# jkrasting/momlevel

Hardware: AMD Instinct MI355X
Metric: Mcells/s for fused Wright-EOS+steric at 1440×1080×75; % HBM roofline (higher is better)
Workload: dtype f64

## Files before the change

momlevel_amd/csrc/build.py:

```python

import os
import shutil
import subprocess
import sys

HERE = os.path.dirname(os.path.abspath(__file__))
PKG = os.path.dirname(HERE)
ROOT = os.path.dirname(PKG)
_TIMED_UNITS = ["momlevel_hip.hip", "momlevel_promote.hip"]
FEATURES = {
    "strat": ["eos_device.hpp", "mlx_internal.hpp", "mlx_pack.hpp"],
    "trend": ["eos_device.hpp", "mlx_internal.hpp", "include/momlevel_trend.h"],
    "clim": ["eos_device.hpp", "mlx_internal.hpp", "mlx_pack.hpp", "include/momlevel_clim.h"],
    "gauge": ["eos_device.hpp", "mlx_internal.hpp", "include/momlevel_gauge.h"],
    "spice": ["mlx_internal.hpp", "include/momlevel_spice.h"],
    "vort": ["mlx_internal.hpp", "include/momlevel_vort.h"],
    "area": ["mlx_internal.hpp", "mlx_pack.hpp", "include/momlevel_area.h"],
    "layer": ["mlx_internal.hpp", "mlx_pack.hpp", "include/momlevel_layer.h"],
    "filter": ["eos_device.hpp", "mlx_internal.hpp", "mlx_pack.hpp", "include/momlevel_filter.h"],
    "quantile": ["eos_device.hpp", "mlx_internal.hpp", "mlx_pack.hpp",
                 "include/momlevel_quantile.h"],
}


def _path(name):
    return os.path.join(ROOT, name) if name.startswith("include/") else os.path.join(HERE, name)


def _feature_files(feature):
    return [_path(f"momlevel_{feature}.hip")] + [_path(name) for name in FEATURES[feature]]


SOURCES = [_path(name) for name in _TIMED_UNITS + [f"momlevel_{f}.hip" for f in FEATURES]
           + ["host_copy.cpp"]]
LIB = os.path.join(PKG, "libmomlevel_hip.so")

FLAGS = [
    "--offload-arch=gfx950",
    "-O3",
    "-ffp-contract=off",
    "-fPIC",
    "-shared",
    "-std=c++17",
    "-Wall",
    "-Wno-unused-variable",
    "-Wno-sometimes-uninitialized",
]


TIMED_SOURCES = [
    os.path.join(HERE, "momlevel_hip.hip"),
    os.path.join(HERE, "eos_device.hpp"),
    os.path.join(HERE, "mlx_internal.hpp"),
    os.path.join(HERE, "momlevel_promote.hip"),
    os.path.join(HERE, "eos_promote.hpp"),
    os.path.join(ROOT, "include", "momlevel_hip.h"),
    os.path.join(ROOT, "include", "momlevel_path.h"),
]
DEPENDS = sorted({*SOURCES, *TIMED_SOURCES, *(p for f in FEATURES for p in _feature_files(f)),
                  os.path.abspath(__file__)})


def source_sha(paths=None, flags=True):
    import hashlib

    h = hashlib.sha256()
    for path in (TIMED_SOURCES if paths is None else paths):
        with open(path, "rb") as f:
            h.update(f.read())
    if flags:
        h.update(" ".join(FLAGS).encode())
    return h.hexdigest()[:16]


def feature_source_sha(feature):
    return source_sha(_feature_files(feature))


def strat_source_sha():
    return feature_source_sha("strat")


def trend_source_sha():
    return feature_source_sha("trend")


def clim_source_sha():
    return feature_source_sha("clim")


def gauge_source_sha():
    return feature_source_sha("gauge")


def spice_source_sha():
    return feature_source_sha("spice")


def vort_source_sha():
    return feature_source_sha("vort")


def area_source_sha():
    return feature_source_sha("area")


def layer_source_sha():
    return feature_source_sha("layer")


def filter_source_sha():
    return feature_source_sha("filter")


def quantile_source_sha():
    return feature_source_sha("quantile")


def hipcc():
    exe = shutil.which("hipcc") or "/opt/rocm/bin/hipcc"
    if not os.path.exists(exe):
        raise RuntimeError("hipcc not found (looked on PATH and in /opt/rocm/bin)")
    return exe


def is_stale():
    if not os.path.exists(LIB):
        return True
    lib_mtime = os.path.getmtime(LIB)
    return any(os.path.getmtime(p) > lib_mtime for p in DEPENDS)


def build(force=False, verbose=False, extra_flags=()):
    if not force and not is_stale():
        return LIB
    cmd = [hipcc()] + FLAGS + list(extra_flags) + SOURCES + ["-o", LIB + ".tmp"]
    if verbose:
        print(" ".join(cmd), flush=True)
    res = subprocess.run(cmd, capture_output=True, text=True)
    if res.returncode != 0:
        raise RuntimeError(f"hipcc failed ({res.returncode}):\n{res.stdout}\n{res.stderr}")
    if verbose and res.stderr:
        print(res.stderr)
    os.replace(LIB + ".tmp", LIB)
    return LIB


if __name__ == "__main__":
    path = build(force="--force" in sys.argv, verbose=True)
    print(path)
```

momlevel_amd/csrc/momlevel_hip.hip:

```cpp

#include <hip/hip_runtime.h>
#include <stdint.h>
#include <stdio.h>
#include <string.h>

#include <initializer_list>
#include <type_traits>

#include "../../include/momlevel_hip.h"
#include "eos_device.hpp"
#include "mlx_internal.hpp"

#pragma clang fp contract(off)

namespace mlx {

constexpr int kBlock = 256;
constexpr int kNTC = 8;

template <typename TIn, int VEC>
struct Pack {
  TIn v[VEC];
};

typedef float f4_t __attribute__((ext_vector_type(4)));

template <bool STREAM>
__device__ __forceinline__ f4_t load16(const void* p) {
  if constexpr (STREAM) return __builtin_nontemporal_load(reinterpret_cast<const f4_t*>(p));
  else return *reinterpret_cast<const f4_t*>(p);
}

template <typename TIn, int VEC, bool STREAM = false>
__device__ __forceinline__ Pack<TIn, VEC> load_pack(const TIn* __restrict__ p) {
  Pack<TIn, VEC> r;
  if constexpr (VEC == 1) {
    if constexpr (STREAM) r.v[0] = __builtin_nontemporal_load(p);
    else r.v[0] = p[0];
  } else if constexpr (sizeof(TIn) * VEC == 8) {
    double raw;
    if constexpr (STREAM) raw = __builtin_nontemporal_load(reinterpret_cast<const double*>(p));
    else raw = *reinterpret_cast<const double*>(p);
    __builtin_memcpy(&r, &raw, 8);
  } else if constexpr (sizeof(TIn) * VEC == 16) {
    f4_t raw = load16<STREAM>(p);
    __builtin_memcpy(&r, &raw, 16);
  } else {
    static_assert(sizeof(TIn) * VEC == 32, "pack must be 16 or 32 bytes");
    f4_t raw0 = load16<STREAM>(p);
    f4_t raw1 = load16<STREAM>(reinterpret_cast<const char*>(p) + 16);
    __builtin_memcpy(&r.v[0], &raw0, 16);
    __builtin_memcpy(&r.v[VEC / 2], &raw1, 16);
  }
  return r;
}

template <int MODE, bool IS_T, typename TIn, int VEC, bool STREAM = false>
__device__ __forceinline__ Pack<TIn, VEC> load_field(const TIn* __restrict__ base, int64_t off) {
  constexpr bool F32_HERE = (MODE == kMixT32 && IS_T) || (MODE == kMixS32 && !IS_T);
  if constexpr (F32_HERE) {
    static_assert((VEC == 1 || VEC == 2) && sizeof(TIn) == 8, "the other field is float64");
    Pack<TIn, VEC> r;
    const float* q = reinterpret_cast<const float*>(base) + off;
    if constexpr (VEC == 2) {
      const Pack<float, 2> f = load_pack<float, 2, STREAM>(q);
      r.v[0] = f.v[0];
      r.v[1] = f.v[1];
    } else if constexpr (STREAM) {
      r.v[0] = __builtin_nontemporal_load(q);
    } else {
      r.v[0] = q[0];
    }
    return r;
  } else {
    return load_pack<TIn, VEC, STREAM>(base + off);
  }
}

__device__ __forceinline__ int64_t xcd_remap(int64_t b, int64_t n) {
  const int64_t q = n / 8, r = n % 8, xcd = b % 8, k = b / 8;
  return (xcd < r ? xcd * (q + 1) : r * (q + 1) + (xcd - r) * q) + k;
}

template <int VEC, bool STREAM = false>
__device__ __forceinline__ void store_pack(double* __restrict__ p, const Pack<double, VEC>& r) {
  if constexpr (VEC == 1) {
    if constexpr (STREAM) __builtin_nontemporal_store(r.v[0], p);
    else p[0] = r.v[0];
  } else {
#pragma unroll
    for (int h = 0; h < VEC / 2; ++h) {
      f4_t raw;
      __builtin_memcpy(&raw, &r.v[2 * h], 16);
      if constexpr (STREAM) __builtin_nontemporal_store(raw, reinterpret_cast<f4_t*>(p) + h);
      else reinterpret_cast<f4_t*>(p)[h] = raw;
    }
  }
}

template <int VEC, bool STREAM = false>
__device__ __forceinline__ void store_pack(float* __restrict__ p, const Pack<float, VEC>& r) {
  if constexpr (VEC == 1) {
    if constexpr (STREAM) __builtin_nontemporal_store(r.v[0], p);
    else p[0] = r.v[0];
  } else if constexpr (VEC == 2) {
    double raw;
    __builtin_memcpy(&raw, &r, 8);
    if constexpr (STREAM) __builtin_nontemporal_store(raw, reinterpret_cast<double*>(p));
    else *reinterpret_cast<double*>(p) = raw;
  } else {
    static_assert(VEC == 4, "float packs are 4, 8 or 16 bytes");
    f4_t raw;
    __builtin_memcpy(&raw, &r, 16);
    if constexpr (STREAM) __builtin_nontemporal_store(raw, reinterpret_cast<f4_t*>(p));
    else *reinterpret_cast<f4_t*>(p) = raw;
  }
}

__device__ __forceinline__ void lds_dma16(const void* gsrc, void* lds_slice) {
#if defined(__HIP_DEVICE_COMPILE__)
  __builtin_amdgcn_global_load_lds(gsrc, (__attribute__((address_space(3))) void*)lds_slice, 16, 0,
                                   2 );
#endif
}

__device__ __forceinline__ double wave_sum(double v) {
#pragma unroll
  for (int off = 32; off > 0; off >>= 1) v += __shfl_down(v, off, 64);
  return v;
}

constexpr int kVarSteric = 0, kVarHalo = 1, kVarThermo = 2, kVarAll = 3;

template <typename TIn, int VEC, int U, int VAR, int MODE, bool GENERIC, bool SKIP, bool FMA,
          bool P3D = false>
__global__ __launch_bounds__(kBlock) void k_steric_global(
    const TIn* __restrict__ T, const TIn* __restrict__ S, const TIn* __restrict__ T0,
    const TIn* __restrict__ S0, const double* __restrict__ vol0, const double* __restrict__ p,
    int p_mode, int eos, int nt, int t_chunk, int64_t plane, int64_t t_stride_T,
    int64_t t_stride_S, double* __restrict__ partials, int64_t nblk_total) {
  constexpr int NOUT = (VAR == kVarAll) ? 4 : 1;
  constexpr int NTC = (VAR == kVarAll) ? kNTC / 2 : kNTC;
  constexpr bool STREAM_T = (VAR != kVarHalo), STREAM_S = (VAR != kVarThermo);
  constexpr bool HELD_T = (VAR == kVarHalo || VAR == kVarAll);
  constexpr bool HELD_S = (VAR == kVarThermo || VAR == kVarAll);
  typedef typename PolyType<MODE>::type R;
  typedef typename PolyVec<MODE, GENERIC ? 1 : VEC>::type RV;
  constexpr int W = Lanes<RV>::n, G = VEC / W;
  constexpr bool GUARD = !GENERIC && VAR != kVarAll;
  constexpr bool PRED = !(VAR == kVarSteric && sizeof(TIn) == 8);
  typedef typename std::conditional<
      FMA, typename FusedFor<MODE>::type,
      typename std::conditional<GUARD, typename ExactFastFor<MODE>::type, ExactOps>::type>::type Ops;
  __shared__ double red[NOUT][NTC][kBlock];

  const int tid = threadIdx.x;
  const int z = blockIdx.y;
  const int nz = gridDim.y;
  const int tb = blockIdx.z * t_chunk;
  const int te = (tb + t_chunk < nt) ? (tb + t_chunk) : nt;
  const int64_t bx = xcd_remap(blockIdx.x, gridDim.x);
  const int64_t blk = (int64_t)blockIdx.y * gridDim.x + bx;
  const int64_t tile0 = bx * (kBlock * VEC * U);
  const int64_t zoff = (int64_t)z * plane;

  int64_t off[U];
  double vol[U][VEC];
  double pc[U][VEC];
  bool alive[U];
#pragma unroll
  for (int u = 0; u < U; ++u) {
    int64_t i = tile0 + ((int64_t)u * kBlock + tid) * VEC;
    const bool valid = (i + VEC <= plane);
    i = valid ? i : 0;
    off[u] = zoff + i;
    Pack<double, VEC> v = load_pack<double, VEC>(vol0 + off[u]);
    bool any_wet = false;
#pragma unroll
    for (int k = 0; k < VEC; ++k) {
      vol[u][k] = valid ? v.v[k] : canonical_nan();
      if constexpr (Ops::contracts && MLX_TUNE_FMA_ACC)
        vol[u][k] = (vol[u][k] == 0.0) ? canonical_nan() : vol[u][k];
      any_wet = any_wet || !is_nan(vol[u][k]);
    }
    alive[u] = !SKIP || any_wet;
    if ((GENERIC && p_mode == MLX_P_FULL3D) || P3D) {
      Pack<double, VEC> q = load_pack<double, VEC>(p + off[u]);
#pragma unroll
      for (int k = 0; k < VEC; ++k) pc[u][k] = q.v[k];
    }
  }
  static_assert(!(P3D && GENERIC), "P3D is the fast kernels' form of MLX_P_FULL3D");
  static_assert(!Ops::fused || W == 1, "pressure folding is per cell");
  double pz = 0.0;
  if ((!GENERIC && !P3D) || p_mode == MLX_P_ZPROF) pz = p[z];
  if (GENERIC && p_mode == MLX_P_SCALAR) pz = p[0];
  auto p_at = [&](int u, int k) -> double { return P3D ? pc[u][k] : pz; };
  auto pfold_at = [&](int u, int g) -> RV {
    RV f = RV{};
    if constexpr (Ops::fused) f = (R)p_at(u, g * W);
    return f;
  };
  lanemask_t pbad[U];
#pragma unroll
  for (int u = 0; u < U; ++u) {
    pbad[u] = P3D ? 0 : Ops::p_unsafe(pz);
    if constexpr (P3D) {
#pragma unroll
      for (int k = 0; k < VEC; ++k) pbad[u] |= Ops::p_unsafe_lanes(pc[u][k]);
    }
  }

  TPart<RV> t0p[(HELD_T && !GENERIC) ? U : 1][G];
  SPart<RV> s0p[(HELD_S && !GENERIC) ? U : 1][G];
  TIn t0v[(HELD_T && GENERIC) ? U : 1][VEC], s0v[(HELD_S && GENERIC) ? U : 1][VEC];
  if constexpr (HELD_T) {
#pragma unroll
    for (int u = 0; u < U; ++u) {
      Pack<TIn, VEC> h = {};
      if (alive[u]) h = load_field<MODE, true, TIn, VEC, true>(T0, off[u]);
#pragma unroll
      for (int k = 0; k < VEC; ++k) {
        if constexpr (GENERIC) t0v[u][k] = h.v[k];
      }
      if constexpr (!GENERIC) {
#pragma unroll
        for (int g = 0; g < G; ++g) t0p[u][g] = t_part_m<MODE, Ops, RV>(Lanes<RV>::make(&h.v[g * W]));
      }
    }
  }
  if constexpr (HELD_S) {
#pragma unroll
    for (int u = 0; u < U; ++u) {
      Pack<TIn, VEC> h = {};
      if (alive[u]) h = load_field<MODE, false, TIn, VEC, true>(S0, off[u]);
#pragma unroll
      for (int k = 0; k < VEC; ++k) {
        if constexpr (GENERIC) s0v[u][k] = h.v[k];
      }
      if constexpr (!GENERIC) {
#pragma unroll
        for (int g = 0; g < G; ++g)
          s0p[u][g] = s_part_m<MODE, Ops, RV>(Lanes<RV>::make(&h.v[g * W]), pfold_at(u, g));
      }
    }
  }

  constexpr bool PREFETCH = !(VAR == kVarAll && sizeof(TIn) == 8 && !GENERIC);
  constexpr bool GLDS = !PREFETCH && !IsMixed<MODE>::value;
  constexpr bool DIRECT = !PREFETCH && !GLDS;
  static_assert(!GLDS || sizeof(TIn) * VEC == 16, "one 16-byte LDS-DMA per pack");
  __shared__ f4_t stage[GLDS ? 2 * U : 1][kBlock];
  Pack<TIn, VEC> curT[U], curS[U], nxtT[PREFETCH ? U : 1], nxtS[PREFETCH ? U : 1];
  if constexpr (GLDS) {
#pragma unroll
    for (int u = 0; u < U; ++u) {
      if (alive[u]) {
        lds_dma16(T + (int64_t)tb * t_stride_T + off[u], &stage[u][tid & ~63]);
        lds_dma16(S + (int64_t)tb * t_stride_S + off[u], &stage[U + u][tid & ~63]);
      }
    }
  }
#pragma unroll
  for (int u = 0; u < (PREFETCH ? U : 0); ++u) {
    nxtT[u] = {};
    nxtS[u] = {};
    if (alive[u]) {
      if (STREAM_T) nxtT[u] = load_field<MODE, true, TIn, VEC, true>(T, (int64_t)tb * t_stride_T + off[u]);
      if (STREAM_S) nxtS[u] = load_field<MODE, false, TIn, VEC, true>(S, (int64_t)tb * t_stride_S + off[u]);
    }
  }

  for (int t = tb; t < te; ++t) {
    if constexpr (GLDS) {
      asm volatile("s_waitcnt vmcnt(0)" ::: "memory");
#pragma unroll
      for (int u = 0; u < U; ++u) {
        __builtin_memcpy(&curT[u], &stage[u][tid], 16);
        __builtin_memcpy(&curS[u], &stage[U + u][tid], 16);
      }
      asm volatile("s_waitcnt lgkmcnt(0)" ::: "memory");
      if (t + 1 < te) {
#pragma unroll
        for (int u = 0; u < U; ++u) {
          if (alive[u]) {
            lds_dma16(T + (int64_t)(t + 1) * t_stride_T + off[u], &stage[u][tid & ~63]);
            lds_dma16(S + (int64_t)(t + 1) * t_stride_S + off[u], &stage[U + u][tid & ~63]);
          }
        }
      }
    }
#pragma unroll
    for (int u = 0; u < (PREFETCH ? U : 0); ++u) {
      if (STREAM_T) curT[u] = nxtT[u];
      if (STREAM_S) curS[u] = nxtS[u];
    }
    if constexpr (DIRECT) {
#pragma unroll
      for (int u = 0; u < U; ++u) {
        curT[u] = {};
        curS[u] = {};
        if (alive[u]) {
          curT[u] = load_field<MODE, true, TIn, VEC, true>(T, (int64_t)t * t_stride_T + off[u]);
          curS[u] = load_field<MODE, false, TIn, VEC, true>(S, (int64_t)t * t_stride_S + off[u]);
        }
      }
    }
    if (PREFETCH && t + 1 < te) {
#pragma unroll
      for (int u = 0; u < U; ++u) {
        if (alive[u]) {
          if (STREAM_T)
            nxtT[u] = load_field<MODE, true, TIn, VEC, true>(T, (int64_t)(t + 1) * t_stride_T + off[u]);
          if (STREAM_S)
            nxtS[u] = load_field<MODE, false, TIn, VEC, true>(S, (int64_t)(t + 1) * t_stride_S + off[u]);
        }
      }
    }
    double c[NOUT];
#pragma unroll
    for (int o = 0; o < NOUT; ++o) c[o] = 0.0;
#pragma unroll
    for (int u = 0; u < U; ++u) {
      if (SKIP && !alive[u]) continue;
      constexpr int NR = NOUT > 1 ? 3 : 1;
      double rho[NR][VEC];
      if constexpr (GENERIC) {
#pragma unroll
        for (int k = 0; k < VEC; ++k) {
          double pp = pz;
          if (p_mode == MLX_P_FULL3D) pp = pc[u][k];
          if (p_mode == MLX_P_FULL4D) pp = p[((int64_t)t * nz) * plane + off[u] + k];
          const TIn tv = STREAM_T ? curT[u].v[k] : t0v[u][k];
          const TIn sv = STREAM_S ? curS[u].v[k] : s0v[u][k];
          rho[0][k] = eos_eval<MODE, TIn, Ops>(eos, kDensity, tv, sv, pp);
          if constexpr (VAR == kVarAll) {
            rho[1][k] = eos_eval<MODE, TIn, Ops>(eos, kDensity, tv, s0v[u][k], pp);
            rho[2][k] = eos_eval<MODE, TIn, Ops>(eos, kDensity, t0v[u][k], sv, pp);
          }
        }
      } else if constexpr (VAR == kVarAll) {
#pragma unroll
        for (int g = 0; g < G; ++g) {
          const TPart<RV> a = t_part_m<MODE, Ops, RV>(Lanes<RV>::make(&curT[u].v[g * W]));
          const SPart<RV> b = s_part_m<MODE, Ops, RV>(Lanes<RV>::make(&curS[u].v[g * W]), pfold_at(u, g));
          double r3[3][W];
          static_assert(!(P3D && VAR == kVarAll), "the all-variants kernel has no register to spare");
          wright_combine_lanes<Ops, RV>(a, b, pz, r3[0]);
          wright_combine_lanes<Ops, RV>(a, s0p[u][g], pz, r3[1]);
          wright_combine_lanes<Ops, RV>(t0p[u][g], b, pz, r3[2]);
#pragma unroll
          for (int w = 0; w < W; ++w) {
            const int k = g * W + w;
#pragma unroll
            for (int o = 0; o < 3; ++o) accumulate<Ops, PRED>(c[o], r3[o][w], vol[u][k]);
            accumulate<ExactOps, PRED>(c[3], (double)curT[u].v[k], vol[u][k]);
          }
        }
        continue;
      } else {
        double num[VEC], den[VEC];
#pragma unroll
        for (int g = 0; g < G; ++g) {
          TPart<RV> a;
          SPart<RV> b;
          if constexpr (STREAM_T) a = t_part_m<MODE, Ops, RV>(Lanes<RV>::make(&curT[u].v[g * W]));
          if constexpr (STREAM_S)
            b = s_part_m<MODE, Ops, RV>(Lanes<RV>::make(&curS[u].v[g * W]), pfold_at(u, g));
          double pg[W];
#pragma unroll
          for (int w = 0; w < W; ++w) pg[w] = p_at(u, g * W + w);
          if constexpr (VAR == kVarSteric)
            wright_numden_lanes<Ops, RV>(a, b, pg, &num[g * W], &den[g * W]);
          if constexpr (VAR == kVarHalo)
            wright_numden_lanes<Ops, RV>(t0p[u][g], b, pg, &num[g * W], &den[g * W]);
          if constexpr (VAR == kVarThermo)
            wright_numden_lanes<Ops, RV>(a, s0p[u][g], pg, &num[g * W], &den[g * W]);
        }
        quotients<Ops, VEC>(num, den, rho[0], pbad[u]);
      }
#pragma unroll
      for (int k = 0; k < VEC; ++k) {
#pragma unroll
        for (int o = 0; o < NR; ++o) accumulate<Ops, PRED>(c[o], rho[o][k], vol[u][k]);
        if constexpr (VAR == kVarAll)
          accumulate<ExactOps, PRED>(c[3], (double)curT[u].v[k], vol[u][k]);
      }
    }
    const int row = (t - tb) % NTC;
#pragma unroll
    for (int o = 0; o < NOUT; ++o) red[o][row][tid] = c[o];
    if (row == NTC - 1 || t == te - 1) {
      __syncthreads();
      const int wave = tid >> 6, lane = tid & 63;
      for (int q = wave; q < NOUT * (row + 1); q += kBlock / 64) {
        const int o = q / (row + 1), r = q % (row + 1);
        double v = ((red[o][r][lane] + red[o][r][lane + 64]) + red[o][r][lane + 128]) +
                   red[o][r][lane + 192];
        v = wave_sum(v);
        if (lane == 0) partials[((int64_t)o * nt + (t - row + r)) * nblk_total + blk] = v;
      }
      __syncthreads();
    }
  }
}

__global__ __launch_bounds__(kBlock) void k_reduce_rows(const double* __restrict__ partials,
                                                        int64_t n, double* __restrict__ out) {
  __shared__ double red[kBlock];
  const double* row = partials + (int64_t)blockIdx.x * n;
  double c = 0.0;
  int64_t i = threadIdx.x;
  for (; i + 7 * (int64_t)kBlock < n; i += 8 * (int64_t)kBlock) {
    double v[8];
#pragma unroll
    for (int k = 0; k < 8; ++k) v[k] = row[i + (int64_t)k * kBlock];
#pragma unroll
    for (int k = 0; k < 8; ++k) c += v[k];
  }
  for (; i < n; i += kBlock) c += row[i];
  red[threadIdx.x] = c;
  __syncthreads();
#pragma unroll
  for (int s = kBlock / 2; s > 0; s >>= 1) {
    if (threadIdx.x < s) red[threadIdx.x] += red[threadIdx.x + s];
    __syncthreads();
  }
  if (threadIdx.x == 0) out[blockIdx.x] = red[0];
}

__global__ __launch_bounds__(kBlock) void k_masso_partial(const double* __restrict__ rho,
                                                          const double* __restrict__ vol,
                                                          int64_t n3, int64_t vol_t_stride,
                                                          double* __restrict__ partials) {
  __shared__ double red[kBlock / 64];
  const int64_t t = blockIdx.y;
  const double* r = rho + t * n3;
  const double* v = vol + t * vol_t_stride;
  double c = 0.0;
  for (int64_t i = (int64_t)blockIdx.x * kBlock + threadIdx.x; i < n3;
       i += (int64_t)gridDim.x * kBlock) {
    const double term = r[i] * v[i];
    c += is_nan(term) ? 0.0 : term;
  }
  c = wave_sum(c);
  if ((threadIdx.x & 63) == 0) red[threadIdx.x >> 6] = c;
  __syncthreads();
  if (threadIdx.x == 0)
    partials[t * gridDim.x + blockIdx.x] = ((red[0] + red[1]) + red[2]) + red[3];
}

template <bool VEC2>
__global__ __launch_bounds__(kBlock) void k_nansum_partial(const double* __restrict__ x, int64_t n,
                                                           double* __restrict__ partials) {
  __shared__ double red[kBlock / 64];
  double c = 0.0;
  if constexpr (VEC2) {
    const int64_t n2 = n / 2;
    double c1 = 0.0;
    for (int64_t i = (int64_t)blockIdx.x * kBlock + threadIdx.x; i < n2;
         i += (int64_t)gridDim.x * kBlock) {
      const Pack<double, 2> v = load_pack<double, 2, true>(x + 2 * i);
      c += is_nan(v.v[0]) ? 0.0 : v.v[0];
      c1 += is_nan(v.v[1]) ? 0.0 : v.v[1];
    }
    c += c1;
  } else {
    for (int64_t i = (int64_t)blockIdx.x * kBlock + threadIdx.x; i < n;
         i += (int64_t)gridDim.x * kBlock) {
      const double v = x[i];
      c += is_nan(v) ? 0.0 : v;
    }
  }
  c = wave_sum(c);
  if ((threadIdx.x & 63) == 0) red[threadIdx.x >> 6] = c;
  __syncthreads();
  if (threadIdx.x == 0) partials[blockIdx.x] = ((red[0] + red[1]) + red[2]) + red[3];
}

constexpr int64_t kProbeMaxBlocks = (int64_t)1 << 23;
constexpr int64_t kK2MaxBlocks1D = ((int64_t)1 << 24) - 1;
template <typename TIn, int NIN, bool WRITE, int U, bool NTS, int VEC = 16 / sizeof(TIn)>
__global__ __launch_bounds__(kBlock) void k_stream_probe_mix(const TIn* __restrict__ a,
                                                             const TIn* __restrict__ b,
                                                             int64_t npacks,
                                                             double* __restrict__ out) {
  double sink = 0.0;
  const int64_t ntiles = (npacks + kBlock * U - 1) / (kBlock * U);
  for (int64_t tile = blockIdx.x; tile < ntiles; tile += gridDim.x) {
    const int64_t base = tile * (kBlock * U) + threadIdx.x;
    Pack<TIn, VEC> x[U], y[U];
#pragma unroll
    for (int u = 0; u < U; ++u) {
      const int64_t i = base + (int64_t)u * kBlock;
      if (i < npacks) {
        x[u] = load_pack<TIn, VEC, true>(a + VEC * i);
        if constexpr (NIN == 2) y[u] = load_pack<TIn, VEC, true>(b + VEC * i);
      }
    }
#pragma unroll
    for (int u = 0; u < U; ++u) {
      const int64_t i = base + (int64_t)u * kBlock;
      if (i < npacks) {
        Pack<double, VEC> r;
#pragma unroll
        for (int k = 0; k < VEC; ++k) {
          r.v[k] = (double)x[u].v[k];
          if constexpr (NIN == 2) r.v[k] += (double)y[u].v[k];
        }
        if constexpr (WRITE) {
          store_pack<VEC, NTS>(out + VEC * i, r);
        } else {
#pragma unroll
          for (int k = 0; k < VEC; ++k) sink += r.v[k];
        }
      }
    }
  }
  if constexpr (!WRITE) {
    if (sink == 0x1.23456789abcdep+1000) out[0] = sink;
  }
}

constexpr int kValuProbeBlocks = 8192;
__global__ __launch_bounds__(kBlock) void k_valu_probe(double* __restrict__ out, int iters,
                                                       double x, double y) {
  double a[8];
#pragma unroll
  for (int k = 0; k < 8; ++k) a[k] = (double)(threadIdx.x + k);
  for (int i = 0; i < iters; ++i) {
#pragma unroll
    for (int k = 0; k < 8; ++k) a[k] = __builtin_fma(a[k], x, y);
  }
  double sink = 0.0;
#pragma unroll
  for (int k = 0; k < 8; ++k) sink += a[k];
  if (sink == 0x1.23456789abcdep+1000) out[0] = sink;
}

template <typename TIn, int VEC, int U, int MODE, int FUNC, bool GENERIC, bool FMA = false,
          bool P3D = false>
__global__ __launch_bounds__(kBlock) void k_eos_map(const TIn* __restrict__ T,
                                                    const TIn* __restrict__ S,
                                                    const double* __restrict__ p, int p_mode,
                                                    int eos, int func, int64_t nz, int64_t plane,
                                                    int64_t t_stride_T, int64_t t_stride_S,
                                                    int64_t t_base, double aux,
                                                    double* __restrict__ out) {
  typedef typename std::conditional<
      FMA, typename FusedFor<MODE>::type,
      typename std::conditional<!GENERIC && FUNC == kDensity, typename ExactFastFor<MODE>::type,
                                ExactOps>::type>::type Ops;
  const int z = blockIdx.y;
  const int64_t t = t_base + blockIdx.z;
  const int64_t tile0 = (int64_t)blockIdx.x * (kBlock * VEC * U);
  const int64_t zoff = (int64_t)z * plane;
  double pz = 0.0;
  if ((!GENERIC && !P3D) || p_mode == MLX_P_ZPROF) pz = p[z];
  if (GENERIC && p_mode == MLX_P_SCALAR) pz = p[0];
  Pack<TIn, VEC> a[U], b[U];
  Pack<double, VEC> pq[U];
  int64_t off[U];
  bool valid[U];
#pragma unroll
  for (int u = 0; u < U; ++u) {
    const int64_t i = tile0 + ((int64_t)u * kBlock + threadIdx.x) * VEC;
    valid[u] = (i + VEC <= plane);
    off[u] = zoff + (valid[u] ? i : 0);
    a[u] = load_pack<TIn, VEC, true>(T + t * t_stride_T + off[u]);
    b[u] = load_pack<TIn, VEC, true>(S + t * t_stride_S + off[u]);
    if constexpr (P3D) pq[u] = load_pack<double, VEC>(p + off[u]);
  }
#pragma unroll
  for (int u = 0; u < U; ++u) {
    Pack<double, VEC> r;
    if constexpr (GENERIC) {
#pragma unroll
      for (int k = 0; k < VEC; ++k) {
        double pp = pz;
        if (p_mode == MLX_P_FULL3D) pp = p[off[u] + k];
        if (p_mode == MLX_P_FULL4D) pp = p[t * nz * plane + off[u] + k];
        r.v[k] = eos_eval<MODE, TIn, Ops>(eos, func, a[u].v[k], b[u].v[k], pp, aux);
      }
    } else if constexpr (FUNC == kDensity) {
      typedef typename PolyType<MODE>::type R;
      typedef typename PolyVec<MODE, VEC>::type RV;
      constexpr int W = Lanes<RV>::n;
      static_assert(!Ops::fused || W == 1, "pressure folding is per cell");
      double num[VEC], den[VEC];
      lanemask_t pbad = P3D ? 0 : Ops::p_unsafe(pz);
#pragma unroll
      for (int k = 0; k < VEC; k += W) {
        double pg[W];
#pragma unroll
        for (int w = 0; w < W; ++w) {
          pg[w] = P3D ? pq[u].v[k + w] : pz;
          if constexpr (P3D) pbad |= Ops::p_unsafe_lanes(pg[w]);
        }
        RV pfold = RV{};
        if constexpr (Ops::fused) pfold = (R)pg[0];
        wright_numden_lanes<Ops, RV>(t_part_m<MODE, Ops, RV>(Lanes<RV>::make(&a[u].v[k])),
                                     s_part_m<MODE, Ops, RV>(Lanes<RV>::make(&b[u].v[k]), pfold), pg,
                                     &num[k], &den[k]);
      }
      quotients<Ops, VEC>(num, den, r.v, pbad);
    } else {
#pragma unroll
      for (int k = 0; k < VEC; ++k)
        r.v[k] = eos_eval<MODE, TIn, Ops>(kWright, FUNC, a[u].v[k], b[u].v[k],
                                          P3D ? pq[u].v[k] : pz);
    }
    if (valid[u]) store_pack<VEC, true>(out + t * nz * plane + off[u], r);
  }
}

__global__ __launch_bounds__(kBlock) void k_fold_mask(const double* __restrict__ rho0,
                                                      const double* __restrict__ vol0, int64_t n,
                                                      double* __restrict__ out) {
  for (int64_t i = (int64_t)blockIdx.x * kBlock + threadIdx.x; i < n;
       i += (int64_t)gridDim.x * kBlock)
    out[i] = is_nan(vol0[i]) ? canonical_nan() : rho0[i];
}

template <typename TIn, int VEC, int NTI, int VAR, int MODE, bool GENERIC, bool SKIP, bool FMA,
          bool P3D = false, bool DRHO32 = false>
__global__ __launch_bounds__(kBlock) void k_steric_local(
    const TIn* __restrict__ T, const TIn* __restrict__ S, const TIn* __restrict__ T0,
    const TIn* __restrict__ S0, const double* __restrict__ rho0m,
    const double* __restrict__ vol0_surface, const double* __restrict__ dz,
    const double* __restrict__ z_i, const double* __restrict__ deptho,
    const double* __restrict__ p, int p_mode, int eos, double neg_inv_rhozero, int nt, int nz,
    int64_t plane, int64_t t_stride_T, int64_t t_stride_S,
    typename std::conditional<DRHO32, float, double>::type* __restrict__ drho_out,
    int64_t drho_vstride, double* __restrict__ eta_out, int64_t eta_vstride, int ntb_major) {
  constexpr int NOUT = (VAR == kVarAll) ? 3 : 1;
  constexpr bool STREAM_T = (VAR != kVarHalo), STREAM_S = (VAR != kVarThermo);
  constexpr bool HELD_T = (VAR == kVarHalo || VAR == kVarAll);
  constexpr bool HELD_S = (VAR == kVarThermo || VAR == kVarAll);
  typedef typename PolyType<MODE>::type R;
  typedef typename PolyVec<MODE, GENERIC ? 1 : VEC>::type RV;
  constexpr int W = Lanes<RV>::n, G = VEC / W;
  typedef typename std::conditional<
      FMA, typename FusedFor<MODE>::type,
      typename std::conditional<GENERIC, ExactOps, typename ExactFastFor<MODE>::type>::type>::type Ops;
  constexpr bool PRED = sizeof(TIn) == 4;
  int64_t tile;
  int tb;
  if (ntb_major > 0) {
    const int64_t q = blockIdx.x >> 3;
    tb = (int)(q % ntb_major);
    tile = (q / ntb_major) * 8 + (blockIdx.x & 7);
  } else {
    tile = xcd_remap(blockIdx.x, gridDim.x);
    tb = blockIdx.y;
  }
  const int64_t col = (tile * kBlock + threadIdx.x) * VEC;
  if (col + VEC > plane) return;
  const int t0 = tb * NTI;
  const int64_t n3 = (int64_t)nz * plane;

  double acc[NOUT][NTI][VEC];
#pragma unroll
  for (int o = 0; o < NOUT; ++o)
#pragma unroll
    for (int j = 0; j < NTI; ++j)
#pragma unroll
      for (int k = 0; k < VEC; ++k) acc[o][j][k] = 0.0;

  Pack<double, VEC> depth;
  if (dz == nullptr) depth = load_pack<double, VEC>(deptho + col);
  double pz = 0.0;
  if (GENERIC && p_mode == MLX_P_SCALAR) pz = p[0];

  Pack<double, VEC> r0n = load_pack<double, VEC>(rho0m + col);

  for (int z = 0; z < nz; ++z) {
    const int64_t off = (int64_t)z * plane + col;
    int64_t sT = t_stride_T, sS = t_stride_S, sD = n3;
    asm volatile("" : "+s"(sT), "+s"(sS), "+s"(sD));
    int64_t oT = (int64_t)t0 * sT, oS = (int64_t)t0 * sS, oD = (int64_t)t0 * sD;
    int nvalid = nt - t0;
    asm volatile("" : "+s"(nvalid));
    const Pack<double, VEC> r0 = r0n;
    if (z + 1 < nz) r0n = load_pack<double, VEC>(rho0m + off + plane);
    Pack<double, VEC> dzv;
    if (dz != nullptr) {
      dzv = load_pack<double, VEC>(dz + off);
    } else {
      const double ztop = z_i[z], zbot = z_i[z + 1];
#pragma unroll
      for (int k = 0; k < VEC; ++k)
        dzv.v[k] = calc_dz_cell<false>(is_nan(depth.v[k]) ? 0.0 : depth.v[k], ztop, zbot, 0.0);
    }
    if ((!GENERIC && !P3D) || p_mode == MLX_P_ZPROF) pz = p[z];
    Pack<double, VEC> pfull;
    if ((GENERIC && p_mode == MLX_P_FULL3D) || P3D) pfull = load_pack<double, VEC>(p + off);
    static_assert(!(P3D && GENERIC), "P3D is the fast kernels' form of MLX_P_FULL3D");
    static_assert(!Ops::fused || W == 1, "pressure folding is per cell");
    lanemask_t pbad = P3D ? 0 : Ops::p_unsafe(pz);
    if constexpr (P3D) {
#pragma unroll
      for (int k = 0; k < VEC; ++k) pbad |= Ops::p_unsafe_lanes(pfull.v[k]);
    }

    bool alive = true;
// ... 1061 lines not shown
```

Baseline: 388,600.

## Peel last time step and add 2-way register rotation in steric time loop

New measurement: 389,500, median of 6. About the same (+0.2%).

```diff
diff --git a/momlevel_amd/csrc/build.py b/momlevel_amd/csrc/build.py
--- a/momlevel_amd/csrc/build.py
+++ b/momlevel_amd/csrc/build.py
@@ -50,6 +50,7 @@
 
 TIMED_SOURCES = [
     os.path.join(HERE, "momlevel_hip.hip"),
+    os.path.join(HERE, "k1_step.hpp"),
     os.path.join(HERE, "eos_device.hpp"),
     os.path.join(HERE, "mlx_internal.hpp"),
     os.path.join(HERE, "momlevel_promote.hip"),
diff --git a/momlevel_amd/csrc/k1_step.hpp b/momlevel_amd/csrc/k1_step.hpp
--- /dev/null
+++ b/momlevel_amd/csrc/k1_step.hpp
@@ -0,0 +1,97 @@
+#ifndef K1_CT
+#define K1_CT curT
+#define K1_CS curS
+#endif
+{
+    const int ts = (K1_T);
+    const bool last = (K1_LAST);
+    double c[NOUT];
+#pragma unroll
+    for (int o = 0; o < NOUT; ++o) c[o] = 0.0;
+#pragma unroll
+    for (int u = 0; u < U; ++u) {
+      if (SKIP && !alive[u]) continue;
+      constexpr int NR = NOUT > 1 ? 3 : 1;
+      double rho[NR][VEC];
+      if constexpr (GENERIC) {
+#pragma unroll
+        for (int k = 0; k < VEC; ++k) {
+          double pp = pz;
+          if (p_mode == MLX_P_FULL3D) pp = pc[u][k];
+          if (p_mode == MLX_P_FULL4D) pp = p[((int64_t)ts * nz) * plane + off[u] + k];
+          const TIn tv = STREAM_T ? K1_CT[u].v[k] : t0v[u][k];
+          const TIn sv = STREAM_S ? K1_CS[u].v[k] : s0v[u][k];
+          rho[0][k] = eos_eval<MODE, TIn, Ops>(eos, kDensity, tv, sv, pp);
+          if constexpr (VAR == kVarAll) {
+            rho[1][k] = eos_eval<MODE, TIn, Ops>(eos, kDensity, tv, s0v[u][k], pp);
+            rho[2][k] = eos_eval<MODE, TIn, Ops>(eos, kDensity, t0v[u][k], sv, pp);
+          }
+        }
+      } else if constexpr (VAR == kVarAll) {
+#pragma unroll
+        for (int g = 0; g < G; ++g) {
+          const TPart<RV> a = t_part_m<MODE, Ops, RV>(Lanes<RV>::make(&K1_CT[u].v[g * W]));
+          const SPart<RV> b = s_part_m<MODE, Ops, RV>(Lanes<RV>::make(&K1_CS[u].v[g * W]), pfold_at(u, g));
+          double r3[3][W];
+          static_assert(!(P3D && VAR == kVarAll), "the all-variants kernel has no register to spare");
+          wright_combine_lanes<Ops, RV>(a, b, pz, r3[0]);
+          wright_combine_lanes<Ops, RV>(a, s0p[u][g], pz, r3[1]);
+          wright_combine_lanes<Ops, RV>(t0p[u][g], b, pz, r3[2]);
+#pragma unroll
+          for (int w = 0; w < W; ++w) {
+            const int k = g * W + w;
+#pragma unroll
+            for (int o = 0; o < 3; ++o) accumulate<Ops, PRED>(c[o], r3[o][w], vol[u][k]);
+            accumulate<ExactOps, PRED>(c[3], (double)K1_CT[u].v[k], vol[u][k]);
+          }
+        }
+        continue;
+      } else {
+        double num[VEC], den[VEC];
+#pragma unroll
+        for (int g = 0; g < G; ++g) {
+          TPart<RV> a;
+          SPart<RV> b;
+          if constexpr (STREAM_T) a = t_part_m<MODE, Ops, RV>(Lanes<RV>::make(&K1_CT[u].v[g * W]));
+          if constexpr (STREAM_S)
+            b = s_part_m<MODE, Ops, RV>(Lanes<RV>::make(&K1_CS[u].v[g * W]), pfold_at(u, g));
+          double pg[W];
+#pragma unroll
+          for (int w = 0; w < W; ++w) pg[w] = p_at(u, g * W + w);
+          if constexpr (VAR == kVarSteric)
+            wright_numden_lanes<Ops, RV>(a, b, pg, &num[g * W], &den[g * W]);
+          if constexpr (VAR == kVarHalo)
+            wright_numden_lanes<Ops, RV>(t0p[u][g], b, pg, &num[g * W], &den[g * W]);
+          if constexpr (VAR == kVarThermo)
+            wright_numden_lanes<Ops, RV>(a, s0p[u][g], pg, &num[g * W], &den[g * W]);
+        }
+        quotients<Ops, VEC>(num, den, rho[0], pbad[u]);
+      }
+#pragma unroll
+      for (int k = 0; k < VEC; ++k) {
+#pragma unroll
+        for (int o = 0; o < NR; ++o) accumulate<Ops, PRED>(c[o], rho[o][k], vol[u][k]);
+        if constexpr (VAR == kVarAll)
+          accumulate<ExactOps, PRED>(c[3], (double)K1_CT[u].v[k], vol[u][k]);
+      }
+    }
+    const int row = (ts - tb) % NTC;
+#pragma unroll
+    for (int o = 0; o < NOUT; ++o) red[o][row][tid] = c[o];
+    if (row == NTC - 1 || last) {
+      __syncthreads();
+      const int wave = tid >> 6, lane = tid & 63;
+      for (int q = wave; q < NOUT * (row + 1); q += kBlock / 64) {
+        const int o = q / (row + 1), r = q % (row + 1);
+        double v = ((red[o][r][lane] + red[o][r][lane + 64]) + red[o][r][lane + 128]) +
+                   red[o][r][lane + 192];
+        v = wave_sum(v);
+        if (lane == 0) partials[((int64_t)o * nt + (ts - row + r)) * nblk_total + blk] = v;
+      }
+      __syncthreads();
+    }
+}
+#undef K1_T
+#undef K1_LAST
+#undef K1_CT
+#undef K1_CS
diff --git a/momlevel_amd/csrc/momlevel_hip.hip b/momlevel_amd/csrc/momlevel_hip.hip
--- a/momlevel_amd/csrc/momlevel_hip.hip
+++ b/momlevel_amd/csrc/momlevel_hip.hip
@@ -131,6 +131,24 @@
 }
 
 constexpr int kVarSteric = 0, kVarHalo = 1, kVarThermo = 2, kVarAll = 3;
+
+constexpr int kK1LoopOne = 0, kK1LoopPeel = 1, kK1LoopRot2 = 2;
+#ifndef MLX_TUNE_K1_LOOP
+#define MLX_TUNE_K1_LOOP -1
+#endif
+constexpr char kK1LoopTable[5][4][9] = {
+    {"00000000", "22212120", "22111211", "00000000"},
+    {"00000000", "02120212", "22122122", "00100000"},
+    {"00000000", "02120221", "22222122", "20102000"},
+    {"00000000", "22002100", "22000200", "00000000"},
+    {"00000000", "22002000", "22001200", "00000000"},
+};
+template <int VAR, int MODE, bool GENERIC, bool SKIP, bool FMA, bool P3D>
+constexpr int k1_loop_form() {
+  if (MLX_TUNE_K1_LOOP >= 0) return MLX_TUNE_K1_LOOP;
+  if (GENERIC) return kK1LoopOne;
+  return kK1LoopTable[MODE][VAR][4 * SKIP + 2 * FMA + P3D] - '0';
+}
 
 template <typename TIn, int VEC, int U, int VAR, int MODE, bool GENERIC, bool SKIP, bool FMA,
           bool P3D = false>
@@ -251,6 +269,8 @@
   constexpr bool DIRECT = !PREFETCH && !GLDS;
   static_assert(!GLDS || sizeof(TIn) * VEC == 16, "one 16-byte LDS-DMA per pack");
   __shared__ f4_t stage[GLDS ? 2 * U : 1][kBlock];
+  constexpr int FORM = k1_loop_form<VAR, MODE, GENERIC, SKIP, FMA, P3D>();
+  constexpr bool PEEL = !DIRECT && FORM != kK1LoopOne, ROT2 = PREFETCH && FORM == kK1LoopRot2;
   Pack<TIn, VEC> curT[U], curS[U], nxtT[PREFETCH ? U : 1], nxtS[PREFETCH ? U : 1];
   if constexpr (GLDS) {
 #pragma unroll
@@ -271,8 +291,84 @@
     }
   }
 
-  for (int t = tb; t < te; ++t) {
-    if constexpr (GLDS) {
+  if constexpr (!PEEL) {
+    for (int t = tb; t < te; ++t) {
+      if constexpr (GLDS) {
+        asm volatile("s_waitcnt vmcnt(0)" ::: "memory");
+#pragma unroll
+        for (int u = 0; u < U; ++u) {
+          __builtin_memcpy(&curT[u], &stage[u][tid], 16);
+          __builtin_memcpy(&curS[u], &stage[U + u][tid], 16);
+        }
+        asm volatile("s_waitcnt lgkmcnt(0)" ::: "memory");
+        if (t + 1 < te) {
+#pragma unroll
+          for (int u = 0; u < U; ++u) {
+            if (alive[u]) {
+              lds_dma16(T + (int64_t)(t + 1) * t_stride_T + off[u], &stage[u][tid & ~63]);
+              lds_dma16(S + (int64_t)(t + 1) * t_stride_S + off[u], &stage[U + u][tid & ~63]);
+            }
+          }
+        }
+      }
+#pragma unroll
+      for (int u = 0; u < (PREFETCH ? U : 0); ++u) {
+        if (STREAM_T) curT[u] = nxtT[u];
+        if (STREAM_S) curS[u] = nxtS[u];
+      }
+      if constexpr (DIRECT) {
+#pragma unroll
+        for (int u = 0; u < U; ++u) {
+          curT[u] = {};
+          curS[u] = {};
+          if (alive[u]) {
+            curT[u] = load_field<MODE, true, TIn, VEC, true>(T, (int64_t)t * t_stride_T + off[u]);
+            curS[u] = load_field<MODE, false, TIn, VEC, true>(S, (int64_t)t * t_stride_S + off[u]);
+          }
+        }
+      }
+      if (PREFETCH && t + 1 < te) {
+#pragma unroll
+        for (int u = 0; u < U; ++u) {
+          if (alive[u]) {
+            if (STREAM_T)
+              nxtT[u] = load_field<MODE, true, TIn, VEC, true>(T, (int64_t)(t + 1) * t_stride_T + off[u]);
+            if (STREAM_S)
+              nxtS[u] = load_field<MODE, false, TIn, VEC, true>(S, (int64_t)(t + 1) * t_stride_S + off[u]);
+          }
+        }
+      }
+#define K1_T t
+#define K1_LAST t == te - 1
+#include "k1_step.hpp"
+    }
+  } else {
+    auto fetch = [&](int t, Pack<TIn, VEC>* dT, Pack<TIn, VEC>* dS) __attribute__((always_inline)) {
+#pragma unroll
+      for (int u = 0; u < U; ++u) {
+        if (alive[u]) {
+          if (STREAM_T) dT[u] = load_field<MODE, true, TIn, VEC, true>(T, (int64_t)t * t_stride_T + off[u]);
+          if (STREAM_S) dS[u] = load_field<MODE, false, TIn, VEC, true>(S, (int64_t)t * t_stride_S + off[u]);
+        }
+      }
+    };
+    auto rotate = [&]() __attribute__((always_inline)) {
+#pragma unroll
+      for (int u = 0; u < (PREFETCH ? U : 0); ++u) {
+        if (STREAM_T) curT[u] = nxtT[u];
+        if (STREAM_S) curS[u] = nxtS[u];
+      }
+    };
+    auto fetch_lds = [&](int t) __attribute__((always_inline)) {
+#pragma unroll
+      for (int u = 0; u < U; ++u) {
+        if (alive[u]) {
+          lds_dma16(T + (int64_t)t * t_stride_T + off[u], &stage[u][tid & ~63]);
+          lds_dma16(S + (int64_t)t * t_stride_S + off[u], &stage[U + u][tid & ~63]);
+        }
+      }
+    };
+    auto read_lds = [&]() __attribute__((always_inline)) {
       asm volatile("s_waitcnt vmcnt(0)" ::: "memory");
 #pragma unroll
       for (int u = 0; u < U; ++u) {
@@ -280,127 +376,57 @@
         __builtin_memcpy(&curS[u], &stage[U + u][tid], 16);
       }
       asm volatile("s_waitcnt lgkmcnt(0)" ::: "memory");
+    };
+    int t = tb;
+    if constexpr (GLDS) {
+      for (; t < te - 1; ++t) {
+        read_lds();
+        fetch_lds(t + 1);
+#define K1_T t
+#define K1_LAST false
+#include "k1_step.hpp"
+      }
+      read_lds();
+#define K1_T t
+#define K1_LAST true
+#include "k1_step.hpp"
+    } else if constexpr (ROT2) {
+      rotate();
+      for (; t + 2 < te; t += 2) {
+        fetch(t + 1, nxtT, nxtS);
+#define K1_T t
+#define K1_LAST false
+#include "k1_step.hpp"
+        fetch(t + 2, curT, curS);
+#define K1_T t + 1
+#define K1_LAST false
+#define K1_CT nxtT
+#define K1_CS nxtS
+#include "k1_step.hpp"
+      }
       if (t + 1 < te) {
-#pragma unroll
-        for (int u = 0; u < U; ++u) {
-          if (alive[u]) {
-            lds_dma16(T + (int64_t)(t + 1) * t_stride_T + off[u], &stage[u][tid & ~63]);
-            lds_dma16(S + (int64_t)(t + 1) * t_stride_S + off[u], &stage[U + u][tid & ~63]);
-          }
-        }
-      }
-    }
-#pragma unroll
-    for (int u = 0; u < (PREFETCH ? U : 0); ++u) {
-      if (STREAM_T) curT[u] = nxtT[u];
-      if (STREAM_S) curS[u] = nxtS[u];
-    }
-    if constexpr (DIRECT) {
-#pragma unroll
-      for (int u = 0; u < U; ++u) {
-        curT[u] = {};
-        curS[u] = {};
-        if (alive[u]) {
-          curT[u] = load_field<MODE, true, TIn, VEC, true>(T, (int64_t)t * t_stride_T + off[u]);
-          curS[u] = load_field<MODE, false, TIn, VEC, true>(S, (int64_t)t * t_stride_S + off[u]);
-        }
-      }
-    }
-    if (PREFETCH && t + 1 < te) {
-#pragma unroll
-      for (int u = 0; u < U; ++u) {
-        if (alive[u]) {
-          if (STREAM_T)
-            nxtT[u] = load_field<MODE, true, TIn, VEC, true>(T, (int64_t)(t + 1) * t_stride_T + off[u]);
-          if (STREAM_S)
-            nxtS[u] = load_field<MODE, false, TIn, VEC, true>(S, (int64_t)(t + 1) * t_stride_S + off[u]);
-        }
-      }
-    }
-    double c[NOUT];
-#pragma unroll
-    for (int o = 0; o < NOUT; ++o) c[o] = 0.0;
-#pragma unroll
-    for (int u = 0; u < U; ++u) {
-      if (SKIP && !alive[u]) continue;
-      constexpr int NR = NOUT > 1 ? 3 : 1;
-      double rho[NR][VEC];
-      if constexpr (GENERIC) {
-#pragma unroll
-        for (int k = 0; k < VEC; ++k) {
-          double pp = pz;
-          if (p_mode == MLX_P_FULL3D) pp = pc[u][k];
-          if (p_mode == MLX_P_FULL4D) pp = p[((int64_t)t * nz) * plane + off[u] + k];
-          const TIn tv = STREAM_T ? curT[u].v[k] : t0v[u][k];
-          const TIn sv = STREAM_S ? curS[u].v[k] : s0v[u][k];
-          rho[0][k] = eos_eval<MODE, TIn, Ops>(eos, kDensity, tv, sv, pp);
-          if constexpr (VAR == kVarAll) {
-            rho[1][k] = eos_eval<MODE, TIn, Ops>(eos, kDensity, tv, s0v[u][k], pp);
-            rho[2][k] = eos_eval<MODE, TIn, Ops>(eos, kDensity, t0v[u][k], sv, pp);
-          }
-        }
-      } else if constexpr (VAR == kVarAll) {
-#pragma unroll
-        for (int g = 0; g < G; ++g) {
-          const TPart<RV> a = t_part_m<MODE, Ops, RV>(Lanes<RV>::make(&curT[u].v[g * W]));
-          const SPart<RV> b = s_part_m<MODE, Ops, RV>(Lanes<RV>::make(&curS[u].v[g * W]), pfold_at(u, g));
-          double r3[3][W];
-          static_assert(!(P3D && VAR == kVarAll), "the all-variants kernel has no register to spare");
-          wright_combine_lanes<Ops, RV>(a, b, pz, r3[0]);
-          wright_combine_lanes<Ops, RV>(a, s0p[u][g], pz, r3[1]);
-          wright_combine_lanes<Ops, RV>(t0p[u][g], b, pz, r3[2]);
-#pragma unroll
-          for (int w = 0; w < W; ++w) {
-            const int k = g * W + w;
-#pragma unroll
-            for (int o = 0; o < 3; ++o) accumulate<Ops, PRED>(c[o], r3[o][w], vol[u][k]);
-            accumulate<ExactOps, PRED>(c[3], (double)curT[u].v[k], vol[u][k]);
-          }
-        }
-        continue;
-      } else {
-        double num[VEC], den[VEC];
-#pragma unroll
-        for (int g = 0; g < G; ++g) {
-          TPart<RV> a;
-          SPart<RV> b;
-          if constexpr (STREAM_T) a = t_part_m<MODE, Ops, RV>(Lanes<RV>::make(&curT[u].v[g * W]));
-          if constexpr (STREAM_S)
-            b = s_part_m<MODE, Ops, RV>(Lanes<RV>::make(&curS[u].v[g * W]), pfold_at(u, g));
-          double pg[W];
-#pragma unroll
-          for (int w = 0; w < W; ++w) pg[w] = p_at(u, g * W + w);
-          if constexpr (VAR == kVarSteric)
-            wright_numden_lanes<Ops, RV>(a, b, pg, &num[g * W], &den[g * W]);
-          if constexpr (VAR == kVarHalo)
-            wright_numden_lanes<Ops, RV>(t0p[u][g], b, pg, &num[g * W], &den[g * W]);
-          if constexpr (VAR == kVarThermo)
-            wright_numden_lanes<Ops, RV>(a, s0p[u][g], pg, &num[g * W], &den[g * W]);
-        }
-        quotients<Ops, VEC>(num, den, rho[0], pbad[u]);
-      }
-#pragma unroll
-      for (int k = 0; k < VEC; ++k) {
-#pragma unroll
-        for (int o = 0; o < NR; ++o) accumulate<Ops, PRED>(c[o], rho[o][k], vol[u][k]);
-        if constexpr (VAR == kVarAll)
-          accumulate<ExactOps, PRED>(c[3], (double)curT[u].v[k], vol[u][k]);
-      }
-    }
-    const int row = (t - tb) % NTC;
-#pragma unroll
-    for (int o = 0; o < NOUT; ++o) red[o][row][tid] = c[o];
-    if (row == NTC - 1 || t == te - 1) {
-      __syncthreads();
-      const int wave = tid >> 6, lane = tid & 63;
-      for (int q = wave; q < NOUT * (row + 1); q += kBlock / 64) {
-        const int o = q / (row + 1), r = q % (row + 1);
-        double v = ((red[o][r][lane] + red[o][r][lane + 64]) + red[o][r][lane + 128]) +
-                   red[o][r][lane + 192];
-        v = wave_sum(v);
-        if (lane == 0) partials[((int64_t)o * nt + (t - row + r)) * nblk_total + blk] = v;
-      }
-      __syncthreads();
+        fetch(t + 1, nxtT, nxtS);
+#define K1_T t
+#define K1_LAST false
+#include "k1_step.hpp"
+        rotate();
+        ++t;
+      }
+#define K1_T t
+#define K1_LAST true
+#include "k1_step.hpp"
+    } else {
+      for (; t < te - 1; ++t) {
+        rotate();
+        fetch(t + 1, nxtT, nxtS);
+#define K1_T t
+#define K1_LAST false
+#include "k1_step.hpp"
+      }
+      rotate();
+#define K1_T t
+#define K1_LAST true
+#include "k1_step.hpp"
     }
   }
 }
```
